# ElBaldo1/FastOptSolver

Measured on AMD Instinct MI355X. Metric: fista_iterations_per_second, higher is better.
Workload: dtype f32

## Files before the change

### fastoptsolver_amd/csrc/cluster_pass.hpp

```cpp
#pragma once
#include "batch_trial.hpp"

namespace fos {

constexpr int CP_ROWS = 16;
constexpr int CP_W = 1024;
constexpr int CP_ASTRIDE = CP_W + 4;
constexpr int CP_THREADS = 320;
constexpr int CP_SLOTS = 4;
constexpr int CP_FLAG_STRIDE = 32;
constexpr unsigned CP_SPIN_LIMIT = 1u << 18;
constexpr size_t CP_LDS_BYTES = (size_t)2 * CP_ROWS * CP_ASTRIDE * 4 + 4 * 64 * 16 + 2 * 64 * 16 + 16;

typedef unsigned long long cp_u64;
__device__ inline void cp_store_sc1(cp_u64* p, cp_u64 v) { __hip_atomic_store(p, v, __ATOMIC_RELAXED, __HIP_MEMORY_SCOPE_AGENT); }
__device__ inline cp_u64 cp_load_sc1(const cp_u64* p) { return __hip_atomic_load(p, __ATOMIC_RELAXED, __HIP_MEMORY_SCOPE_AGENT); }
__device__ inline cp_u64 cp_pack(float lo, float hi) { return ((cp_u64)__float_as_uint(hi) << 32) | __float_as_uint(lo); }

template <int CS, int MODE = 0>
__global__ __launch_bounds__(CP_THREADS) void cluster_pass_kernel(const float* __restrict__ A, int64_t lda,
                                                                 const float* __restrict__ b, int64_t m, int n, int n_pad,
                                                                 const float* __restrict__ xp, int64_t rows_per_cluster,
                                                                 int xcd_aware, float* __restrict__ xchg,
                                                                 unsigned* __restrict__ flags, unsigned epoch,
                                                                 float* __restrict__ slabs, int64_t n_stride,
                                                                 int* __restrict__ error) {
  extern __shared__ __attribute__((aligned(16))) char cp_lds[];
  float (*a_s)[CP_ROWS][CP_ASTRIDE] = reinterpret_cast<float (*)[CP_ROWS][CP_ASTRIDE]>(cp_lds);
  f32x4 (*red)[64] = reinterpret_cast<f32x4 (*)[64]>(cp_lds + (size_t)2 * CP_ROWS * CP_ASTRIDE * 4);
  f32x4 (*r_s)[64] = reinterpret_cast<f32x4 (*)[64]>(cp_lds + (size_t)2 * CP_ROWS * CP_ASTRIDE * 4 + 4 * 64 * 16);
  int* abort_s = reinterpret_cast<int*>(cp_lds + (size_t)2 * CP_ROWS * CP_ASTRIDE * 4 + 4 * 64 * 16 + 2 * 64 * 16);

  const int tid = threadIdx.x, lane = tid & 63, wave = tid >> 6;
  const bool mc = wave < 4;
  int cluster, member;
  if (xcd_aware) {
    const int xcd = blockIdx.x % 8, idx = blockIdx.x / 8;
    cluster = xcd + 8 * (idx / CS);
    member = idx % CS;
  } else {
    cluster = blockIdx.x / CS;
    member = blockIdx.x % CS;
  }
  const int col_strip = member * CP_W;
  const int64_t row_lo = (int64_t)cluster * rows_per_cluster;
  const int npanels = (int)(rows_per_cluster / CP_ROWS);
  if (tid == 0) *abort_s = 0;

  f32x4 xr[16];
  f32x4 G[16];
  f32x4 areg[CP_ROWS];
  const int wcol = col_strip + 256 * (wave & 3);
  if (mc) {
#pragma unroll
    for (int s = 0; s < 16; ++s) {
      const int col = wcol + 16 * s;
      const f32x4 v = *reinterpret_cast<const f32x4*>(xp + ((int64_t)((col < n_pad ? col : 0) / 16) * 4 + (lane >> 4)) * 64 +
                                                      (lane & 15) * 4);
      xr[s] = col < n_pad ? v : f32x4{0.f, 0.f, 0.f, 0.f};
      G[s] = f32x4{0.f, 0.f, 0.f, 0.f};
    }
  }
  int lcol = col_strip + 4 * tid;
  if (lcol >= n) lcol = n - 4;
  auto load_tile = [&](int pnl) {
    if ((MODE & 4) && pnl >= 2) return;
    if (pnl >= npanels) pnl = npanels - 1;
#pragma unroll
    for (int u = 0; u < CP_ROWS; ++u) {
      int64_t row = row_lo + (int64_t)pnl * CP_ROWS + u;
      if (row >= m) row = m - 1;
      areg[u] = __builtin_nontemporal_load(reinterpret_cast<const f32x4*>(A + row * lda + lcol));
    }
  };
  auto store_tile = [&](int buf) {
#pragma unroll
    for (int u = 0; u < CP_ROWS; ++u) *reinterpret_cast<f32x4*>(&a_s[buf][u][4 * tid]) = areg[u];
  };

  if (mc) {
    load_tile(0);
    store_tile(0);
    load_tile(1);
  }
  __syncthreads();

  for (int i = 0; i <= npanels; ++i) {
    if (mc) {
      if (i < npanels) {
        const int buf = i & 1;
        f32x4 acc = {0.f, 0.f, 0.f, 0.f}, acc_odd = {0.f, 0.f, 0.f, 0.f};
#pragma unroll
        for (int s = 0; s < ((MODE & 2) ? 1 : 16); ++s) {
          const f32x4 a4 = *reinterpret_cast<const f32x4*>(&a_s[buf][lane & 15][256 * wave + 16 * s + 4 * (lane >> 4)]);
          acc = __builtin_amdgcn_mfma_f32_16x16x4f32(a4.x, xr[s].x, acc, 0, 0, 0);
          acc_odd = __builtin_amdgcn_mfma_f32_16x16x4f32(a4.y, xr[s].y, acc_odd, 0, 0, 0);
          acc = __builtin_amdgcn_mfma_f32_16x16x4f32(a4.z, xr[s].z, acc, 0, 0, 0);
          acc_odd = __builtin_amdgcn_mfma_f32_16x16x4f32(a4.w, xr[s].w, acc_odd, 0, 0, 0);
        }
        red[wave][lane] = acc + acc_odd;
      }
    } else if (i >= 1 && (MODE & 1)) {
      r_s[(i - 1) & 1][lane] = red[0][lane];
    } else if (i >= 1) {
      const int q = i - 1;
      bool ok = true;
      if (lane < CS) {
        const unsigned* f = flags + ((size_t)cluster * CS + lane) * CP_FLAG_STRIDE;
        unsigned spins = 0;
        while ((int)(__hip_atomic_load(f, __ATOMIC_RELAXED, __HIP_MEMORY_SCOPE_AGENT) - epoch) < q + 1) {
          if (++spins > CP_SPIN_LIMIT) { ok = false; break; }
          __builtin_amdgcn_s_sleep(1);
        }
      }
      if (__ballot(!ok) != 0) {
        if (lane == 0) { *abort_s = 1; *error = 1; }
      } else {
        constexpr int GC = CS < 8 ? CS : 8;
        f32x4 r = {0.f, 0.f, 0.f, 0.f};
#pragma unroll 1
        for (int j0 = 0; j0 < CS; j0 += GC) {
          cp_u64 lo[GC], hi[GC];
#pragma unroll
          for (int j = 0; j < GC; ++j) {
            const cp_u64* src = reinterpret_cast<const cp_u64*>(
                xchg + (((size_t)cluster * CP_SLOTS + (q % CP_SLOTS)) * CS + j0 + j) * 256 + lane * 4);
            lo[j] = cp_load_sc1(src);
            hi[j] = cp_load_sc1(src + 1);
          }
#pragma unroll
          for (int j = 0; j < GC; ++j) {
            r.x += __uint_as_float((unsigned)lo[j]); r.y += __uint_as_float((unsigned)(lo[j] >> 32));
            r.z += __uint_as_float((unsigned)hi[j]); r.w += __uint_as_float((unsigned)(hi[j] >> 32));
          }
        }
        const int64_t row0 = row_lo + (int64_t)q * CP_ROWS + 4 * (lane >> 4);
        float rv[4] = {r.x, r.y, r.z, r.w};
#pragma unroll
        for (int c = 0; c < 4; ++c) {
          const int64_t row = row0 + c;
          rv[c] = row < m ? (b != nullptr ? rv[c] - b[row] : rv[c]) : 0.f;
        }
        r_s[q & 1][lane] = f32x4{rv[0], rv[1], rv[2], rv[3]};
      }
    }
    __syncthreads();
    if (*abort_s) break;
    if (mc) {
      if (i >= 1) {
        const int buf = (i - 1) & 1;
        const f32x4 r4 = r_s[(i - 1) & 1][lane];
        const float rc[4] = {r4.x, r4.y, r4.z, r4.w};
#pragma unroll
        for (int c = 0; c < ((MODE & 2) ? 1 : 4); ++c) {
#pragma unroll
          for (int t = 0; t < 16; ++t)
            G[t] = __builtin_amdgcn_mfma_f32_16x16x4f32(rc[c], a_s[buf][4 * (lane >> 4) + c][256 * wave + 16 * t + (lane & 15)],
                                                        G[t], 0, 0, 0);
        }
      }
    } else if (i < npanels && !(MODE & 1)) {
      const f32x4 s = ((red[0][lane] + red[1][lane]) + red[2][lane]) + red[3][lane];
      cp_u64* dst = reinterpret_cast<cp_u64*>(xchg + (((size_t)cluster * CP_SLOTS + (i % CP_SLOTS)) * CS + member) * 256 + lane * 4);
      cp_store_sc1(dst, cp_pack(s.x, s.y));
      cp_store_sc1(dst + 1, cp_pack(s.z, s.w));
      asm volatile("s_waitcnt vmcnt(0)" ::: "memory");
      if (lane == 0)
        __hip_atomic_store(flags + ((size_t)cluster * CS + member) * CP_FLAG_STRIDE, epoch + (unsigned)i + 1u, __ATOMIC_RELAXED,
                           __HIP_MEMORY_SCOPE_AGENT);
    }
    __syncthreads();
    if (mc && i + 1 < npanels) {
      store_tile((i + 1) & 1);
      load_tile(i + 2);
    }
    __syncthreads();
  }

  if (mc && *abort_s == 0) {
#pragma unroll
    for (int t = 0; t < 16; ++t) {
      const int col = wcol + 16 * t + (lane & 15);
      if (col < n) {
        const float gv[4] = {G[t].x, G[t].y, G[t].z, G[t].w};
#pragma unroll
        for (int r = 0; r < 4; ++r) slabs[((int64_t)cluster * BT_NV + 4 * (lane >> 4) + r) * n_stride + col] = gv[r];
      }
    }
  }
}

}
```

Baseline: 105.0.

## Emulate fp32 MFMA with split-bf16 products and double compute waves

Replaces the fp32 16x16x4 MFMA matvecs in both the A*x and A^T*r phases with a three-way bf16 split (hi/mid/lo) using six bf16 MFMAs per block. This is meant to use the much higher bf16 matrix throughput while keeping close to fp32 accuracy. It also doubles the compute waves from 4 to 8 per block, with narrower column strips and fewer tile rows loaded per thread, and stores the residual in LDS as pre-split bf16. The costs are extra VALU work for splitting, more MFMA instructions, a small loss of accuracy from dropping the lowest-order cross terms, and higher register and LDS pressure.

New measurement: 104.9. No clear change (-0.1%).

```diff
diff --git a/fastoptsolver_amd/csrc/cluster_pass.hpp b/fastoptsolver_amd/csrc/cluster_pass.hpp
--- a/fastoptsolver_amd/csrc/cluster_pass.hpp
+++ b/fastoptsolver_amd/csrc/cluster_pass.hpp
@@ -6,16 +6,53 @@
 constexpr int CP_ROWS = 16;
 constexpr int CP_W = 1024;
 constexpr int CP_ASTRIDE = CP_W + 4;
-constexpr int CP_THREADS = 320;
+constexpr int CP_MCW = 8;
+constexpr int CP_WCOLS = CP_W / CP_MCW;
+constexpr int CP_LROWS = CP_ROWS * (CP_W / 4) / (64 * CP_MCW);
+constexpr int CP_THREADS = 64 * (CP_MCW + 1);
 constexpr int CP_SLOTS = 4;
 constexpr int CP_FLAG_STRIDE = 32;
 constexpr unsigned CP_SPIN_LIMIT = 1u << 18;
-constexpr size_t CP_LDS_BYTES = (size_t)2 * CP_ROWS * CP_ASTRIDE * 4 + 4 * 64 * 16 + 2 * 64 * 16 + 16;
+constexpr size_t CP_RS_BYTES = 2 * 3 * 64 * 8;
+constexpr size_t CP_RED_BYTES = CP_MCW * 64 * 16;
+constexpr size_t CP_LDS_BYTES = (size_t)2 * CP_ROWS * CP_ASTRIDE * 4 + CP_RED_BYTES + CP_RS_BYTES + 16;
 
 typedef unsigned long long cp_u64;
 __device__ inline void cp_store_sc1(cp_u64* p, cp_u64 v) { __hip_atomic_store(p, v, __ATOMIC_RELAXED, __HIP_MEMORY_SCOPE_AGENT); }
 __device__ inline cp_u64 cp_load_sc1(const cp_u64* p) { return __hip_atomic_load(p, __ATOMIC_RELAXED, __HIP_MEMORY_SCOPE_AGENT); }
 __device__ inline cp_u64 cp_pack(float lo, float hi) { return ((cp_u64)__float_as_uint(hi) << 32) | __float_as_uint(lo); }
+
+typedef float cp_f32x2 __attribute__((ext_vector_type(2)));
+typedef unsigned cp_u32x2 __attribute__((ext_vector_type(2)));
+typedef unsigned cp_u32x4 __attribute__((ext_vector_type(4)));
+typedef short cp_bf16x4 __attribute__((ext_vector_type(4)));
+__device__ inline void cp_split2(cp_f32x2 a, unsigned& hi, unsigned& mid, unsigned& lo) {
+  const cp_u32x2 ua = __builtin_bit_cast(cp_u32x2, a);
+  const cp_f32x2 r1 = a - __builtin_bit_cast(cp_f32x2, ua & 0xffff0000u);
+  const cp_u32x2 u1 = __builtin_bit_cast(cp_u32x2, r1);
+  const cp_u32x2 u2 = __builtin_bit_cast(cp_u32x2, r1 - __builtin_bit_cast(cp_f32x2, u1 & 0xffff0000u));
+  hi = __builtin_amdgcn_perm(ua.y, ua.x, 0x07060302u);
+  mid = __builtin_amdgcn_perm(u1.y, u1.x, 0x07060302u);
+  lo = __builtin_amdgcn_perm(u2.y, u2.x, 0x07060302u);
+}
+__device__ inline void cp_split8(f32x4 p, f32x4 q, bf16x8& hi, bf16x8& mid, bf16x8& lo) {
+  unsigned h[4], m[4], l[4];
+  cp_split2(cp_f32x2{p.x, p.y}, h[0], m[0], l[0]);
+  cp_split2(cp_f32x2{p.z, p.w}, h[1], m[1], l[1]);
+  cp_split2(cp_f32x2{q.x, q.y}, h[2], m[2], l[2]);
+  cp_split2(cp_f32x2{q.z, q.w}, h[3], m[3], l[3]);
+  hi = __builtin_bit_cast(bf16x8, cp_u32x4{h[0], h[1], h[2], h[3]});
+  mid = __builtin_bit_cast(bf16x8, cp_u32x4{m[0], m[1], m[2], m[3]});
+  lo = __builtin_bit_cast(bf16x8, cp_u32x4{l[0], l[1], l[2], l[3]});
+}
+__device__ inline void cp_split4(f32x4 p, cp_bf16x4& hi, cp_bf16x4& mid, cp_bf16x4& lo) {
+  unsigned h[2], m[2], l[2];
+  cp_split2(cp_f32x2{p.x, p.y}, h[0], m[0], l[0]);
+  cp_split2(cp_f32x2{p.z, p.w}, h[1], m[1], l[1]);
+  hi = __builtin_bit_cast(cp_bf16x4, cp_u32x2{h[0], h[1]});
+  mid = __builtin_bit_cast(cp_bf16x4, cp_u32x2{m[0], m[1]});
+  lo = __builtin_bit_cast(cp_bf16x4, cp_u32x2{l[0], l[1]});
+}
 
 template <int CS, int MODE = 0>
 __global__ __launch_bounds__(CP_THREADS) void cluster_pass_kernel(const float* __restrict__ A, int64_t lda,
@@ -28,11 +65,11 @@
   extern __shared__ __attribute__((aligned(16))) char cp_lds[];
   float (*a_s)[CP_ROWS][CP_ASTRIDE] = reinterpret_cast<float (*)[CP_ROWS][CP_ASTRIDE]>(cp_lds);
   f32x4 (*red)[64] = reinterpret_cast<f32x4 (*)[64]>(cp_lds + (size_t)2 * CP_ROWS * CP_ASTRIDE * 4);
-  f32x4 (*r_s)[64] = reinterpret_cast<f32x4 (*)[64]>(cp_lds + (size_t)2 * CP_ROWS * CP_ASTRIDE * 4 + 4 * 64 * 16);
-  int* abort_s = reinterpret_cast<int*>(cp_lds + (size_t)2 * CP_ROWS * CP_ASTRIDE * 4 + 4 * 64 * 16 + 2 * 64 * 16);
-
-  const int tid = threadIdx.x, lane = tid & 63, wave = tid >> 6;
-  const bool mc = wave < 4;
+  cp_bf16x4 (*r_s)[3][64] = reinterpret_cast<cp_bf16x4 (*)[3][64]>(cp_lds + (size_t)2 * CP_ROWS * CP_ASTRIDE * 4 + CP_RED_BYTES);
+  int* abort_s = reinterpret_cast<int*>(cp_lds + (size_t)2 * CP_ROWS * CP_ASTRIDE * 4 + CP_RED_BYTES + CP_RS_BYTES);
+
+  const int tid = threadIdx.x, lane = tid & 63, wave = __builtin_amdgcn_readfirstlane(tid >> 6);
+  const bool mc = wave < CP_MCW;
   int cluster, member;
   if (xcd_aware) {
     const int xcd = blockIdx.x % 8, idx = blockIdx.x / 8;
@@ -47,35 +84,38 @@
   const int npanels = (int)(rows_per_cluster / CP_ROWS);
   if (tid == 0) *abort_s = 0;
 
-  f32x4 xr[16];
-  f32x4 G[16];
-  f32x4 areg[CP_ROWS];
-  const int wcol = col_strip + 256 * (wave & 3);
+  bf16x8 yq[CP_WCOLS / 32][3];
+  f32x4 G[CP_WCOLS / 16];
+  f32x4 areg[CP_LROWS];
+  const int wcol = col_strip + CP_WCOLS * (wave & (CP_MCW - 1));
   if (mc) {
 #pragma unroll
-    for (int s = 0; s < 16; ++s) {
-      const int col = wcol + 16 * s;
-      const f32x4 v = *reinterpret_cast<const f32x4*>(xp + ((int64_t)((col < n_pad ? col : 0) / 16) * 4 + (lane >> 4)) * 64 +
-                                                      (lane & 15) * 4);
-      xr[s] = col < n_pad ? v : f32x4{0.f, 0.f, 0.f, 0.f};
-      G[s] = f32x4{0.f, 0.f, 0.f, 0.f};
-    }
-  }
-  int lcol = col_strip + 4 * tid;
+    for (int kb = 0; kb < CP_WCOLS / 32; ++kb) {
+      const int col = wcol + 32 * kb + 8 * (lane >> 4);
+      const float* src = xp + ((int64_t)((col < n_pad ? col : 0) / 16) * 4 + 2 * ((lane >> 4) & 1)) * 64 + (lane & 15) * 4;
+      f32x4 v0 = *reinterpret_cast<const f32x4*>(src), v1 = *reinterpret_cast<const f32x4*>(src + 64);
+      if (col >= n_pad) v0 = v1 = f32x4{0.f, 0.f, 0.f, 0.f};
+      cp_split8(v0, v1, yq[kb][0], yq[kb][1], yq[kb][2]);
+    }
+#pragma unroll
+    for (int t = 0; t < CP_WCOLS / 16; ++t) G[t] = f32x4{0.f, 0.f, 0.f, 0.f};
+  }
+  const int lchunk = tid & 255, lrow = CP_LROWS * ((tid >> 8) & 1);
+  int lcol = col_strip + 4 * lchunk;
   if (lcol >= n) lcol = n - 4;
   auto load_tile = [&](int pnl) {
     if ((MODE & 4) && pnl >= 2) return;
     if (pnl >= npanels) pnl = npanels - 1;
 #pragma unroll
-    for (int u = 0; u < CP_ROWS; ++u) {
-      int64_t row = row_lo + (int64_t)pnl * CP_ROWS + u;
+    for (int u = 0; u < CP_LROWS; ++u) {
+      int64_t row = row_lo + (int64_t)pnl * CP_ROWS + lrow + u;
       if (row >= m) row = m - 1;
       areg[u] = __builtin_nontemporal_load(reinterpret_cast<const f32x4*>(A + row * lda + lcol));
     }
   };
   auto store_tile = [&](int buf) {
 #pragma unroll
-    for (int u = 0; u < CP_ROWS; ++u) *reinterpret_cast<f32x4*>(&a_s[buf][u][4 * tid]) = areg[u];
+    for (int u = 0; u < CP_LROWS; ++u) *reinterpret_cast<f32x4*>(&a_s[buf][lrow + u][4 * lchunk]) = areg[u];
   };
 
   if (mc) {
@@ -89,19 +129,23 @@
     if (mc) {
       if (i < npanels) {
         const int buf = i & 1;
-        f32x4 acc = {0.f, 0.f, 0.f, 0.f}, acc_odd = {0.f, 0.f, 0.f, 0.f};
-#pragma unroll
-        for (int s = 0; s < ((MODE & 2) ? 1 : 16); ++s) {
-          const f32x4 a4 = *reinterpret_cast<const f32x4*>(&a_s[buf][lane & 15][256 * wave + 16 * s + 4 * (lane >> 4)]);
-          acc = __builtin_amdgcn_mfma_f32_16x16x4f32(a4.x, xr[s].x, acc, 0, 0, 0);
-          acc_odd = __builtin_amdgcn_mfma_f32_16x16x4f32(a4.y, xr[s].y, acc_odd, 0, 0, 0);
-          acc = __builtin_amdgcn_mfma_f32_16x16x4f32(a4.z, xr[s].z, acc, 0, 0, 0);
-          acc_odd = __builtin_amdgcn_mfma_f32_16x16x4f32(a4.w, xr[s].w, acc_odd, 0, 0, 0);
-        }
-        red[wave][lane] = acc + acc_odd;
+        f32x4 acc0 = {0.f, 0.f, 0.f, 0.f}, acc1 = {0.f, 0.f, 0.f, 0.f}, acc2 = {0.f, 0.f, 0.f, 0.f};
+        const float* src = &a_s[buf][lane & 15][CP_WCOLS * wave + 8 * (lane >> 4)];
+#pragma unroll
+        for (int kb = 0; kb < ((MODE & 2) ? 1 : CP_WCOLS / 32); ++kb) {
+          bf16x8 ah, am, al;
+          cp_split8(*reinterpret_cast<const f32x4*>(src + 32 * kb), *reinterpret_cast<const f32x4*>(src + 32 * kb + 4), ah, am, al);
+          acc0 = __builtin_amdgcn_mfma_f32_16x16x32_bf16(ah, yq[kb][0], acc0, 0, 0, 0);
+          acc1 = __builtin_amdgcn_mfma_f32_16x16x32_bf16(ah, yq[kb][1], acc1, 0, 0, 0);
+          acc2 = __builtin_amdgcn_mfma_f32_16x16x32_bf16(ah, yq[kb][2], acc2, 0, 0, 0);
+          acc1 = __builtin_amdgcn_mfma_f32_16x16x32_bf16(am, yq[kb][0], acc1, 0, 0, 0);
+          acc2 = __builtin_amdgcn_mfma_f32_16x16x32_bf16(am, yq[kb][1], acc2, 0, 0, 0);
+          acc2 = __builtin_amdgcn_mfma_f32_16x16x32_bf16(al, yq[kb][0], acc2, 0, 0, 0);
+        }
+        red[wave][lane] = (acc2 + acc1) + acc0;
       }
     } else if (i >= 1 && (MODE & 1)) {
-      r_s[(i - 1) & 1][lane] = red[0][lane];
+      cp_split4(red[0][lane], r_s[(i - 1) & 1][0][lane], r_s[(i - 1) & 1][1][lane], r_s[(i - 1) & 1][2][lane]);
     } else if (i >= 1) {
       const int q = i - 1;
       bool ok = true;
@@ -134,14 +178,15 @@
             r.z += __uint_as_float((unsigned)hi[j]); r.w += __uint_as_float((unsigned)(hi[j] >> 32));
           }
         }
-        const int64_t row0 = row_lo + (int64_t)q * CP_ROWS + 4 * (lane >> 4);
+        const int64_t prow = row_lo + (int64_t)q * CP_ROWS;
+        const int left = (int)(m - prow < CP_ROWS ? (m - prow < 0 ? 0 : m - prow) : CP_ROWS);
         float rv[4] = {r.x, r.y, r.z, r.w};
 #pragma unroll
         for (int c = 0; c < 4; ++c) {
-          const int64_t row = row0 + c;
-          rv[c] = row < m ? (b != nullptr ? rv[c] - b[row] : rv[c]) : 0.f;
-        }
-        r_s[q & 1][lane] = f32x4{rv[0], rv[1], rv[2], rv[3]};
+          const int u = 4 * (lane >> 4) + c;
+          rv[c] = u < left ? (b != nullptr ? rv[c] - b[prow + u] : rv[c]) : 0.f;
+        }
+        cp_split4(f32x4{rv[0], rv[1], rv[2], rv[3]}, r_s[q & 1][0][lane], r_s[q & 1][1][lane], r_s[q & 1][2][lane]);
       }
     }
     __syncthreads();
@@ -149,18 +194,48 @@
     if (mc) {
       if (i >= 1) {
         const int buf = (i - 1) & 1;
-        const f32x4 r4 = r_s[(i - 1) & 1][lane];
-        const float rc[4] = {r4.x, r4.y, r4.z, r4.w};
-#pragma unroll
-        for (int c = 0; c < ((MODE & 2) ? 1 : 4); ++c) {
-#pragma unroll
-          for (int t = 0; t < 16; ++t)
-            G[t] = __builtin_amdgcn_mfma_f32_16x16x4f32(rc[c], a_s[buf][4 * (lane >> 4) + c][256 * wave + 16 * t + (lane & 15)],
-                                                        G[t], 0, 0, 0);
+        if constexpr (!(MODE & 8)) {
+          const cp_bf16x4 rh = r_s[buf][0][lane], rm = r_s[buf][1][lane], rl = r_s[buf][2][lane];
+          const float* src = &a_s[buf][4 * (lane >> 4)][CP_WCOLS * wave + (lane & 15)];
+#pragma unroll
+          for (int t = 0; t < ((MODE & 2) ? 1 : CP_WCOLS / 16); ++t) {
+            cp_bf16x4 th, tm, tl;
+            cp_split4(f32x4{src[16 * t], src[16 * t + CP_ASTRIDE], src[16 * t + 2 * CP_ASTRIDE], src[16 * t + 3 * CP_ASTRIDE]}, th, tm, tl);
+            G[t] = __builtin_amdgcn_mfma_f32_16x16x16bf16_1k(rh, th, G[t], 0, 0, 0);
+            G[t] = __builtin_amdgcn_mfma_f32_16x16x16bf16_1k(rh, tm, G[t], 0, 0, 0);
+            G[t] = __builtin_amdgcn_mfma_f32_16x16x16bf16_1k(rm, th, G[t], 0, 0, 0);
+            G[t] = __builtin_amdgcn_mfma_f32_16x16x16bf16_1k(rh, tl, G[t], 0, 0, 0);
+            G[t] = __builtin_amdgcn_mfma_f32_16x16x16bf16_1k(rm, tm, G[t], 0, 0, 0);
+            G[t] = __builtin_amdgcn_mfma_f32_16x16x16bf16_1k(rl, th, G[t], 0, 0, 0);
+          }
+        } else {
+          const int g = (lane >> 4) & 1, w = lane & 15;
+          bf16x8 rq[3];
+#pragma unroll
+          for (int p = 0; p < 3; ++p) {
+            const cp_bf16x4 u = r_s[buf][p][w + 32 * g], v = r_s[buf][p][w + 32 * g + 16];
+            rq[p] = lane < 32 ? bf16x8{u.x, u.y, u.z, u.w, v.x, v.y, v.z, v.w} : bf16x8{0, 0, 0, 0, 0, 0, 0, 0};
+          }
+          const float* src = &a_s[buf][8 * g][CP_WCOLS * wave + w];
+#pragma unroll
+          for (int t = 0; t < ((MODE & 2) ? 1 : CP_WCOLS / 16); ++t) {
+            bf16x8 th, tm, tl;
+            cp_split8(f32x4{src[16 * t], src[16 * t + CP_ASTRIDE], src[16 * t + 2 * CP_ASTRIDE], src[16 * t + 3 * CP_ASTRIDE]},
+                      f32x4{src[16 * t + 4 * CP_ASTRIDE], src[16 * t + 5 * CP_ASTRIDE], src[16 * t + 6 * CP_ASTRIDE],
+                            src[16 * t + 7 * CP_ASTRIDE]}, th, tm, tl);
+            G[t] = __builtin_amdgcn_mfma_f32_16x16x32_bf16(rq[0], th, G[t], 0, 0, 0);
+            G[t] = __builtin_amdgcn_mfma_f32_16x16x32_bf16(rq[0], tm, G[t], 0, 0, 0);
+            G[t] = __builtin_amdgcn_mfma_f32_16x16x32_bf16(rq[1], th, G[t], 0, 0, 0);
+            G[t] = __builtin_amdgcn_mfma_f32_16x16x32_bf16(rq[0], tl, G[t], 0, 0, 0);
+            G[t] = __builtin_amdgcn_mfma_f32_16x16x32_bf16(rq[1], tm, G[t], 0, 0, 0);
+            G[t] = __builtin_amdgcn_mfma_f32_16x16x32_bf16(rq[2], th, G[t], 0, 0, 0);
+          }
         }
       }
     } else if (i < npanels && !(MODE & 1)) {
-      const f32x4 s = ((red[0][lane] + red[1][lane]) + red[2][lane]) + red[3][lane];
+      f32x4 s = red[0][lane];
+#pragma unroll
+      for (int w = 1; w < CP_MCW; ++w) s += red[w][lane];
       cp_u64* dst = reinterpret_cast<cp_u64*>(xchg + (((size_t)cluster * CP_SLOTS + (i % CP_SLOTS)) * CS + member) * 256 + lane * 4);
       cp_store_sc1(dst, cp_pack(s.x, s.y));
       cp_store_sc1(dst + 1, cp_pack(s.z, s.w));
@@ -179,7 +254,7 @@
 
   if (mc && *abort_s == 0) {
 #pragma unroll
-    for (int t = 0; t < 16; ++t) {
+    for (int t = 0; t < CP_WCOLS / 16; ++t) {
       const int col = wcol + 16 * t + (lane & 15);
       if (col < n) {
         const float gv[4] = {G[t].x, G[t].y, G[t].z, G[t].w};
```
